# speedinghzl/DSRG

Measured on AMD Instinct MI355X. Metric: images/sec DSRG train step (VGG16 321x321, 21-class), higher is better.
Workload: dtype bf16 backbone (fp32 master weights) + f32/f64 supervision path

## Files before the change

dsrg_amd/_lib.py:

```python
import ctypes
import os

import torch

_HERE = os.path.dirname(os.path.abspath(__file__))
LIB_PATH = os.path.join(_HERE, os.environ.get("DSRG_LIB") or "libdsrg_hip.so")

OK, ERR_INVALID, ERR_HIP, ERR_UNSUPPORTED, ERR_NOMEM = 0, -1, -2, -3, -4


class DsrgError(RuntimeError):
    def __init__(self, code, msg):
        RuntimeError.__init__(self, "libdsrg_hip error %d: %s" % (code, msg))
        self.code = code


class CrfParams(ctypes.Structure):
    _fields_ = [("w_bilateral", ctypes.c_float), ("theta_alpha_x", ctypes.c_float),
                ("theta_alpha_y", ctypes.c_float), ("theta_beta_r", ctypes.c_float),
                ("theta_beta_g", ctypes.c_float), ("theta_beta_b", ctypes.c_float),
                ("w_gaussian", ctypes.c_float), ("theta_gamma_x", ctypes.c_float),
                ("theta_gamma_y", ctypes.c_float), ("n_iters", ctypes.c_int32)]

    @classmethod
# ... 60 lines not shown
    "dsrg_flush_reductions": (_i, [_vp]),
    "dsrg_conv_igemm_residual_bf16": (_i, [_vp] * 6 + [_i] * 8 + [_vp]),
    "dsrg_conv_igemm_split_f32": (_i, [_vp, _vp, _vp, _vp] + [_i] * 8 + [_vp]),
    "dsrg_add_relu_bf16": (_i, [_vp, _vp, _vp, _sz, _vp]),
    "dsrg_relu_mask_bf16": (_i, [_vp, _vp, _vp, _vp, _sz, _vp]),
    "dsrg_bias_grad_bf16": (_i, [_vp, _vp, _vp, _i, ctypes.c_long, _i, _vp]),
    "dsrg_heads_forward_bf16": (_i, [_vp, _i, _vp, _vp, _vp, _i, _i, _i, _i, _vp]),
    "dsrg_conv3x3_direct_bf16": (_i, [_vp, _vp, _vp, _vp, _i, _i, _i, _i, _i, _i, _vp]),
    "dsrg_conv3x3_direct_dgrad_workspace": (_sz, [_i]),
    "dsrg_conv3x3_direct_dgrad_bf16": (_i, [_vp] * 6 + [_sz] + [_i] * 5 + [_vp]),
    "dsrg_conv_igemm_supported": (_i, [_i, _i, _i]),
    "dsrg_conv_igemm_bf16": (_i, [_vp, _vp, _vp, _vp, _vp, _i, _i, _i, _i, _i, _i, _i, _i, ctypes.c_float, ctypes.c_ulonglong, _vp, _sz,
                                  _vp]),
    "dsrg_conv_igemm_workspace": (_sz, []),
    "dsrg_conv_igemm_dgrad_workspace": (_sz, [_i] * 5),
    "dsrg_conv_igemm_dgrad_bf16": (_i, [_vp] * 6 + [_i] * 7 + [_f, _vp, _sz, _vp]),
    "dsrg_conv_igemm_workspace_status": (_i, [_vp, _vp, _vp]),
    "dsrg_pack_conv_weight_f32": (_i, [_vp, _vp, _vp, _i, _i, _i, _vp]),
    "dsrg_sgd_pack_f32": (_i, [_i] + [_vp] * 9 + [_f, _vp]),
    "dsrg_conv_igemm_wgrad_workspace": (_sz, [_i, _i, _i, _i, _i, _i, _i]),
    "dsrg_conv_igemm_wgrad_bf16": (_i, [_vp, _vp, _vp, _vp, _i, _vp, _sz, _i, _i, _i, _i, _i, _i, _i, _vp]),
    "dsrg_conv_igemm_backward_bf16": (_i, [_vp, _vp, _vp, _vp, _vp, _vp, _i, _vp, _f, _vp, ctypes.c_size_t, _vp, ctypes.c_size_t, _i, _i, _i, _i, _i, _i, _vp]),
    "dsrg_conv3x3_wgrad_workspace": (_sz, [_i, _i, _i, _i, _i]),
    "dsrg_conv3x3_wgrad_bf16": (_i, [_vp, _vp, _vp, _vp, _sz, _i, _i, _i, _i, _i, _vp]),
    "dsrg_conv3x3_wgrad_f32": (_i, [_vp, _vp, _vp, _vp, _sz, _i, _i, _i, _i, _i, _vp]),
    "dsrg_pack_conv_weight_direct_f32": (_i, [_vp, _vp, _vp, _i, _i, _vp]),
    "dsrg_heads_backward_chunks": (_i, [_i]),
    "dsrg_heads_backward_bf16": (_i, [_vp, _i, _vp, _vp, _vp, _sz, _vp, _vp, _i, _i, _i, _i, _vp]),
    "dsrg_heads_backward_relu_workspace": (_sz, [_i] * 3),
    "dsrg_heads_backward_relu_bf16": (_i, [_vp, _i, _vp, _vp, _vp, _sz, _vp, _vp, _f, _vp, _vp, _sz] + [_i] * 4 + [_vp]),
    "dsrg_maxpool3x3_fwd_bf16": (_i, [_vp, _vp, _vp, _i, _i, _i, _i, _i, _i, _i, _vp]),
    "dsrg_maxpool3x3_relu_fwd_bf16": (_i, [_vp, _vp, _vp, _i, _i, _i, _i, _i, _i, _i, _vp]),
    "dsrg_maxpool3x3_bwd_bf16": (_i, [_vp, _vp, _vp, _i, _i, _i, _i, _i, _i, _i, _vp]),
    "dsrg_maxpool3x3_bwd_relu_bf16": (_i, [_vp, _vp, _vp, _vp, _vp, _vp, _i, _i, _i, _i, _i, _i, _i, _vp]),
    "dsrg_supervision_step": (_i, [_vp, _i, _vp, _vp, _i, _i, _vp, _vp, _d, _d, ctypes.POINTER(CrfParams),
                                   _vp, _vp, _vp, _vp, _vp, _vp]),
}

_LIB = None


def lib():
    global _LIB
    if _LIB is None:
        if not os.path.exists(LIB_PATH):
            raise ImportError(
                "%s is missing — build it with `make -C dsrg_amd/csrc` (hipcc --offload-arch=gfx950) or "
                "`python -c 'import __graft_entry__ as g; g.build()'`.  There is no CPU fallback." % LIB_PATH)
        L = ctypes.CDLL(LIB_PATH)
        for name, (res, args) in SIGNATURES.items():
            fn = getattr(L, name)
            fn.restype = res
            fn.argtypes = args
        _LIB = L
    return _LIB


def check(rc):
    if rc != OK:
        raise DsrgError(rc, lib().dsrg_last_error().decode("utf-8", "replace"))


def require_gpu():
    if lib().dsrg_device_count() < 1:
        raise DsrgError(ERR_HIP, "no HIP device visible — the DSRG supervision kernels need an MI355X "
                                 "(gfx950); there is no CPU fallback")
# ... 1 lines not shown
```

dsrg_amd/backbone.py:

```python
import torch
import torch.nn as nn
import torch.nn.functional as F


import os as _os
_WGRAD_MIN_COUT = int(_os.environ.get("DSRG_WGRAD_MIN_COUT", "512"))
_DIRECT_CONV = _os.environ.get("DSRG_DIRECT_CONV", "1")
_DIRECT_C3 = _os.environ.get("DSRG_DIRECT_C3", "1") == "1"
_DIRECT_FN = _os.environ.get("DSRG_DIRECT_FN", "1") == "1"
_FUSE_POOL = _os.environ.get("DSRG_FUSE_POOL", "1") == "1"
_GEMM_1X1_BWD = _os.environ.get("DSRG_GEMM_1X1_BWD", "1") == "1"
_DIRECT_WGRAD = _os.environ.get("DSRG_DIRECT_WGRAD", "1") == "1"
_GEMM_DGRAD_MAX_MAP = int(_os.environ.get("DSRG_GEMM_DGRAD_MAX_MAP", "2048"))
_WGRAD_T = _os.environ.get("DSRG_WGRAD_T", "1") == "1"
_IGEMM = _os.environ.get("DSRG_IGEMM", "1") == "1"
_FC7_IGEMM = _os.environ.get("DSRG_FC7_IGEMM", "1") == "1"


def _im2col_gemm(x, weight, bias, dilation, relu, want_cols=False):
    B, C, H, W = x.shape
    cout, k = weight.shape[0], weight.shape[2]
    xn = x.permute(0, 2, 3, 1)
    if not xn.is_contiguous():
        xn = xn.contiguous()
# ... 434 lines not shown

class FusedDropout(nn.Identity):
    """placeholder for the Dropout layer that runs inside the GemmConv2d two slots in front of it (`fuse_dropout`)"""


class _MaxPool3x3Fn(torch.autograd.Function):
    @staticmethod
    def forward(ctx, x, stride, ceil_mode):
        from .ops import maxpool3x3_fwd
        out, code = maxpool3x3_fwd(x, stride, ceil_mode)
        ctx.save_for_backward(code)
        ctx.in_shape, ctx.stride = x.shape, stride
        return out

    @staticmethod
    def backward(ctx, g):
        from .ops import maxpool3x3_bwd
        (code,) = ctx.saved_tensors
        return maxpool3x3_bwd(g, code, ctx.in_shape, ctx.stride), None, None


class _AvgPool3x3Fn(torch.autograd.Function):
    @staticmethod
    def forward(ctx, x):
        from .ops import avgpool3x3_s1
        return avgpool3x3_s1(x)

    @staticmethod
    def backward(ctx, g):
        from .ops import avgpool3x3_s1
        return avgpool3x3_s1(g)


class AvgPool3x3(nn.AvgPool2d):

    def __init__(self):
        super().__init__(3, 1, 1)

    def forward(self, x):
        if x.is_cuda and x.dtype == torch.bfloat16 and x.shape[1] % 8 == 0 and \
                x.is_contiguous(memory_format=torch.channels_last):
            return _AvgPool3x3Fn.apply(x)
        if x.is_cuda and x.dim() == 4 and not x.is_contiguous():
            x = x.contiguous()
        return super().forward(x)


class MaxPool3x3(nn.MaxPool2d):

    def __init__(self, stride, ceil_mode=False):
        super().__init__(3, stride, 1, ceil_mode=ceil_mode)

    def forward(self, x):
        if x.is_cuda and x.dtype == torch.bfloat16 and x.shape[1] % 8 == 0 and \
                x.is_contiguous(memory_format=torch.channels_last):
            return _MaxPool3x3Fn.apply(x, self.stride, self.ceil_mode)
        return super().forward(x)


def _pool3x3(x, stride, ceil_mode):
    if x.is_cuda and x.dtype == torch.bfloat16 and x.shape[1] % 8 == 0 and x.is_contiguous(memory_format=torch.channels_last):
        return _MaxPool3x3Fn.apply(x, stride, ceil_mode)
    return F.max_pool2d(x, 3, stride, 1, ceil_mode=ceil_mode)


def _conv_relu(cin, cout, dilation=1, gemm=False, pool=None, chain=False):
# ... 39 lines not shown
    @staticmethod
    def backward(ctx, g):
        return tuple(g[i].as_strided(shape, stride) if g[i].is_contiguous() else g[i].reshape(shape)
                     for i, (shape, stride) in enumerate(ctx.layouts))


class VGG16ASPP(nn.Module):

    def __init__(self, num_classes=21, dropout=0.5, gemm_convs=True):
        super().__init__()
        L = []
        p2 = (2, True)
        L += _conv_relu(3, 64) + _conv_relu(64, 64, pool=p2, chain=True)
        L += _conv_relu(64, 128, 1, gemm_convs) + _conv_relu(128, 128, 1, gemm_convs, pool=p2, chain=True)
        L += _conv_relu(128, 256, 1, gemm_convs) + _conv_relu(256, 256, 1, gemm_convs, chain=True) + \
            _conv_relu(256, 256, 1, gemm_convs, pool=p2, chain=True)
        g = gemm_convs
        L += _conv_relu(256, 512, 1, g) + _conv_relu(512, 512, 1, g, chain=True) + _conv_relu(512, 512, 1, g, chain=True) + [MaxPool3x3(1)]
        L += _conv_relu(512, 512, 2, g) + _conv_relu(512, 512, 2, g, chain=True) + _conv_relu(512, 512, 2, g, chain=True) + [MaxPool3x3(1)]
        L += [AvgPool3x3()]
        self.features = nn.Sequential(*L)
        self.branches = nn.ModuleList()
        for d in (6, 12, 18, 24):
            g = gemm_convs
            fc8 = GemmConv2d(1024, num_classes, 1, gemm=g)
            nn.init.normal_(fc8.weight, std=0.01)
            nn.init.zeros_(fc8.bias)
            self.branches.append(nn.Sequential(
                GemmConv2d(512, 1024, 3, padding=d, dilation=d, fuse_relu=True, gemm=g, fuse_dropout=dropout), FusedReLU(),
                FusedDropout(),
                GemmConv2d(1024, 1024, 1, fuse_relu=True, gemm=g, fuse_dropout=dropout), FusedReLU(), FusedDropout(), fc8))

    def forward(self, x):
        f = self.features(x)
        hs = []
        fc6 = [br[0] for br in self.branches]
        if len(fc6) <= 4 and all(_igemm_route(m, f, len(fc6)) and m.stride == (1, 1) and m.padding == m.dilation for m in fc6):
            p = fc6[0].fuse_dropout if self.training else 0.0
            n = len(fc6)
            links = [_GradLink() for _ in range(n)] if torch.is_grad_enabled() else None
            hs = list(_IgemmConvFn.apply(3, [m.dilation[0] for m in fc6], True, p, None, n, None, links, *([f] * n),
                                         *[m.weight for m in fc6], *[m.bias for m in fc6]))
            fc7 = [br[3] for br in self.branches]
            if all(isinstance(m, GemmConv2d) and m.kernel_size == (1, 1) and m.fuse_relu and m.bias is not None and m.gemm
                   and m.in_channels % 256 == 0 and m.out_channels % 256 == 0 for m in fc7):
                p7 = fc7[0].fuse_dropout if self.training else 0.0
                links7 = [_GradLink() for _ in range(n)] if torch.is_grad_enabled() else None
                hs = list(_IgemmConvFn.apply(1, [1] * n, True, p7, None, n, links, links7, *hs, *[m.weight for m in fc7],
                                             *[m.bias for m in fc7]))
                for h, lk in zip(hs, links7 or []):
                    h._dsrg_grad_link = lk
            else:
                for i, br in enumerate(self.branches):
                    for m in list(br)[1:-1]:
                        hs[i] = m(hs[i])
        else:
            for br in self.branches:
                h = f
                for m in list(br)[:-1]:
                    h = m(h)
                hs.append(h)
        heads = [br[-1] for br in self.branches]
        if hs[0].is_cuda and hs[0].dtype == torch.bfloat16 and len(hs) <= 4 and heads[0].out_channels <= 32 \
                and heads[0].in_channels % 256 == 0:
            w = _StackKernels.apply(*[m.weight for m in heads])
            b = torch.stack([m.bias for m in heads])
            links = [getattr(h, "_dsrg_grad_link", None) for h in hs]
# ... 57 lines not shown
```

dsrg_amd/csrc/api.hip:

```cpp
#include <math.h>
#include <stdarg.h>
#include <stdio.h>
#include <string.h>
#include <mutex>
#include <new>
#include "common.h"

namespace dsrg {

static thread_local char g_err[512] = "";
int set_error(int code, const char *fmt, ...) {
    va_list ap;
    va_start(ap, fmt);
    vsnprintf(g_err, sizeof(g_err), fmt, ap);
    va_end(ap);
    return code;
}

static inline size_t align256(size_t x) { return (x + 255) & ~(size_t)255; }

}

using namespace dsrg;

// ... 603 lines not shown
extern "C" int dsrg_heads_backward_chunks(int M) { return heads_bwd_chunks(M); }
extern "C" int dsrg_heads_backward_bf16(const void *const *x_dev, int n_branches, const float *w_dev, const float *g_dev,
                                        void *gx_dev, size_t gx_branch_stride_bytes, float *gw_dev, float *partial_dev, int B,
                                        int HW, int K, int O, void *stream) {
    if (!x_dev || !w_dev || !g_dev || (!gx_dev && !gw_dev) || (gw_dev && !partial_dev) || B < 1 || HW < 1)
        return set_error(DSRG_ERR_INVALID, "bad argument");
    for (int k = 0; k < n_branches && k < 4; k++)
        if (!x_dev[k]) return set_error(DSRG_ERR_INVALID, "NULL branch input");
    return launch_heads_bwd(x_dev, n_branches, w_dev, g_dev, gx_dev, gx_branch_stride_bytes, gw_dev, partial_dev, B, HW, K, O,
                            static_cast<hipStream_t>(stream));
}
extern "C" size_t dsrg_heads_backward_relu_workspace(int n_branches, int M, int K) { return heads_bwd_relu_workspace(n_branches, M, K); }
extern "C" int dsrg_heads_backward_relu_bf16(const void *const *x_dev, int n_branches, const float *w_dev, const float *g_dev,
                                             void *gx_dev, size_t gx_branch_stride_bytes, float *gw_dev, float *partial_dev,
                                             float relu_scale, float *bias_grad_dev, void *workspace_dev, size_t workspace_bytes,
                                             int B, int HW, int K, int O, void *stream) {
    if (!x_dev || !w_dev || !g_dev || !gx_dev || (gw_dev && !partial_dev) || B < 1 || HW < 1 || !(relu_scale > 0.0f) || !bias_grad_dev)
        return set_error(DSRG_ERR_INVALID, "bad argument");
    for (int k = 0; k < n_branches && k < 4; k++)
        if (!x_dev[k]) return set_error(DSRG_ERR_INVALID, "NULL branch input");
    return launch_heads_bwd(x_dev, n_branches, w_dev, g_dev, gx_dev, gx_branch_stride_bytes, gw_dev, partial_dev, B, HW, K, O,
                            static_cast<hipStream_t>(stream), relu_scale, bias_grad_dev, workspace_dev, workspace_bytes);
}
extern "C" int dsrg_maxpool3x3_fwd_bf16(const void *in, void *out, void *code, int B, int H, int W, int OH, int OW, int C,
                                        int stride, void *stream) {
    if (!in || !out || !code) return set_error(DSRG_ERR_INVALID, "NULL argument");
    return launch_maxpool3x3_fwd(in, out, code, B, H, W, OH, OW, C, stride, static_cast<hipStream_t>(stream));
}
extern "C" int dsrg_maxpool3x3_relu_fwd_bf16(const void *in, void *out, void *code, int B, int H, int W, int OH, int OW, int C,
                                             int stride, void *stream) {
    if (!in || !out || !code) return set_error(DSRG_ERR_INVALID, "NULL argument");
    return launch_maxpool3x3_fwd(in, out, code, B, H, W, OH, OW, C, stride, static_cast<hipStream_t>(stream), true);
}
extern "C" int dsrg_maxpool3x3_bwd_bf16(const void *gout, const void *code, void *gin, int B, int H, int W, int OH, int OW,
                                        int C, int stride, void *stream) {
    if (!gout || !code || !gin) return set_error(DSRG_ERR_INVALID, "NULL argument");
    return launch_maxpool3x3_bwd(gout, code, gin, B, H, W, OH, OW, C, stride, static_cast<hipStream_t>(stream));
}

extern "C" int dsrg_maxpool3x3_bwd_relu_bf16(const void *gout, const void *code, const void *relu_out, void *gin, float *bias_grad,
                                             float *partials, int partial_blocks, int B, int H, int W, int OH, int OW, int C,
                                             void *stream) {
    if (!gout || !code || !gin || !bias_grad || !partials) return set_error(DSRG_ERR_INVALID, "NULL argument");
    return launch_maxpool3x3_bwd_relu(gout, code, relu_out, gin, bias_grad, partials, partial_blocks, B, H, W, OH, OW, C,
                                      static_cast<hipStream_t>(stream));
}

extern "C" int dsrg_supervision_step(dsrg_ctx_t c, int B, const float *logits, const float *images, int img_h,
                                     int img_w, const float *labels, const float *cues, double th1, double th2,
                                     const dsrg_crf_params *prm, float *losses, float *grad_logits,
                                     float *probs_out, float *seeds_out, float *logq_out, void *stream) {
    if (!c || !logits || !labels || !cues || !losses || !grad_logits)
        return set_error(DSRG_ERR_INVALID, "NULL argument");
    if (B < 1 || B > c->maxB) return set_error(DSRG_ERR_INVALID, "batch %d outside 1..%d", B, c->maxB);
    const bool prepared = images == nullptr;
    {
        int prc = check_params(prm);
        if (prc) return prc;
    }
    if (!prepared && (img_h < 1 || img_w < 1)) return set_error(DSRG_ERR_INVALID, "bad image size");
    if (prepared) {
        if (c->prepared_B != B || memcmp(&c->prepared_prm, prm, offsetof(dsrg_crf_params, n_iters)) != 0)
            return set_error(DSRG_ERR_INVALID, "images_dev is NULL but dsrg_crf_prepare_batch was not called "
                                               "for this batch size / these kernel parameters");
    }
    hipStream_t s = static_cast<hipStream_t>(stream);
// ... 228 lines not shown
```

dsrg_amd/csrc/backbone_ops.hip:

```cpp
#include "common.h"
#include <algorithm>
#ifndef DSRG_EXP
#define DSRG_EXP 0
#endif
#include <cstdlib>
#include <cstring>

namespace dsrg {

__device__ __forceinline__ float bf16_lo(uint32_t w) { return __uint_as_float(w << 16); }
__device__ __forceinline__ float bf16_hi(uint32_t w) { return __uint_as_float(w & 0xffff0000u); }
__device__ __forceinline__ uint32_t f32_to_bf16_rne(float f) {
    uint32_t u = __float_as_uint(f);
    if ((u & 0x7fffffffu) > 0x7f800000u) return (u >> 16) | 0x40u;
    return (u + 0x7fffu + ((u >> 16) & 1u)) >> 16;
}
__device__ __forceinline__ uint32_t pack_bf16(float lo, float hi) { return f32_to_bf16_rne(lo) | (f32_to_bf16_rne(hi) << 16); }

constexpr int kRbThreads = 256;

__global__ __launch_bounds__(kRbThreads) void relu_bwd_bias_kernel(const uint4 *__restrict__ g, const uint4 *__restrict__ y,
                                                                    uint4 *__restrict__ gm, float *__restrict__ part,
                                                                    int rows, int C8, int rows_per_block, float scale) {
    __shared__ float red[kRbThreads][9];
// ... 320 lines not shown
    size_t r = idx / C8;
    const int x = (int)(r % W);
    r /= W;
    const int y = (int)(r % H);
    const int b = (int)(r / H);
    float acc[8] = {0.f, 0.f, 0.f, 0.f, 0.f, 0.f, 0.f, 0.f};
#pragma unroll
    for (int dy = -1; dy <= 1; ++dy) {
        const int yy = y + dy;
        if (yy < 0 || yy >= H) continue;
#pragma unroll
        for (int dx = -1; dx <= 1; ++dx) {
            const int xx = x + dx;
            if (xx < 0 || xx >= W) continue;
            const uint4 v = in[(((size_t)b * H + yy) * W + xx) * C8 + c];
            const uint32_t w[4] = {v.x, v.y, v.z, v.w};
#pragma unroll
            for (int k = 0; k < 4; ++k) { acc[2 * k] += bf16_lo(w[k]); acc[2 * k + 1] += bf16_hi(w[k]); }
        }
    }
#pragma unroll
    for (int k = 0; k < 8; ++k) acc[k] = acc[k] / 9.0f;
    out[idx] = make_uint4(pack_bf16(acc[0], acc[1]), pack_bf16(acc[2], acc[3]), pack_bf16(acc[4], acc[5]), pack_bf16(acc[6], acc[7]));
}
int launch_avgpool3x3_s1(const void *in, void *out, int B, int H, int W, int C, hipStream_t stream) {
    if (C % 8 != 0) return set_error(DSRG_ERR_UNSUPPORTED, "avgpool3x3: channels must be a multiple of 8");
    if (B <= 0 || H <= 0 || W <= 0) return set_error(DSRG_ERR_INVALID, "avgpool3x3: bad shape");
    const size_t total = (size_t)B * H * W * (C / 8);
    hipLaunchKernelGGL(avgpool3x3_s1_kernel, dim3((unsigned)((total + 255) / 256)), dim3(256), 0, stream, (const uint4 *)in,
                       (uint4 *)out, B, H, W, C / 8);
    DSRG_LAUNCH_CHECK();
    return DSRG_OK;
}

__global__ __launch_bounds__(256) void add_relu_kernel(const uint4 *__restrict__ a, const uint4 *__restrict__ b, uint4 *__restrict__ y, size_t n8) {
    const size_t i = (size_t)blockIdx.x * 256 + threadIdx.x;
    if (i >= n8) return;
    const uint4 va = a[i], vb = b[i];
    const uint32_t wa[4] = {va.x, va.y, va.z, va.w}, wb[4] = {vb.x, vb.y, vb.z, vb.w};
    uint32_t o[4];
#pragma unroll
    for (int k = 0; k < 4; k++)
        o[k] = pack_bf16(fmaxf(bf16_lo(wa[k]) + bf16_lo(wb[k]), 0.0f), fmaxf(bf16_hi(wa[k]) + bf16_hi(wb[k]), 0.0f));
    y[i] = make_uint4(o[0], o[1], o[2], o[3]);
}
__global__ __launch_bounds__(256) void relu_mask_kernel(const uint4 *__restrict__ g, const uint4 *__restrict__ g2, const uint4 *__restrict__ y,
                                                        uint4 *__restrict__ gm, size_t n8) {
    const size_t i = (size_t)blockIdx.x * 256 + threadIdx.x;
    if (i >= n8) return;
    const uint4 vg = g[i], vy = y[i];
    uint32_t wg[4] = {vg.x, vg.y, vg.z, vg.w};
    const uint32_t wy[4] = {vy.x, vy.y, vy.z, vy.w};
    if (g2) {
        const uint4 v2 = g2[i];
        const uint32_t w2[4] = {v2.x, v2.y, v2.z, v2.w};
#pragma unroll
        for (int k = 0; k < 4; k++) wg[k] = pack_bf16(bf16_lo(wg[k]) + bf16_lo(w2[k]), bf16_hi(wg[k]) + bf16_hi(w2[k]));
    }
#pragma unroll
    for (int k = 0; k < 4; k++)
        wg[k] &= ((int16_t)(wy[k] & 0xffffu) > 0 ? 0x0000ffffu : 0u) | ((int32_t)wy[k] >= 0x10000 ? 0xffff0000u : 0u);
    gm[i] = make_uint4(wg[0], wg[1], wg[2], wg[3]);
}
int launch_add_relu(const void *a, const void *b, void *y, size_t n, hipStream_t stream) {
    if (n == 0 || n % 8) return set_error(DSRG_ERR_INVALID, "add_relu: element count must be a positive multiple of 8");
    hipLaunchKernelGGL(add_relu_kernel, dim3((unsigned)((n / 8 + 255) / 256)), dim3(256), 0, stream, (const uint4 *)a, (const uint4 *)b,
// ... 787 lines not shown
```

dsrg_amd/csrc/common.h:

```cpp
#pragma once
#include <hip/hip_runtime.h>
#include <stdint.h>
#include <stddef.h>
#include <atomic>
#include "../../include/dsrg_hip.h"

namespace dsrg {

int set_error(int code, const char *fmt, ...);
#define DSRG_HIP_CHECK(expr)                                                              \
    do {                                                                                  \
        hipError_t _e = (expr);                                                           \
        if (_e != hipSuccess)                                                             \
            return ::dsrg::set_error(DSRG_ERR_HIP, "%s failed: %s (%s:%d)", #expr,        \
                                     hipGetErrorString(_e), __FILE__, __LINE__);          \
    } while (0)
#define DSRG_LAUNCH_CHECK() DSRG_HIP_CHECK(hipGetLastError())

__device__ __forceinline__ void colsum_block(const float *__restrict__ p, float *__restrict__ out, int rows, int cout, int bx, float (*red)[64]) {
    const int cl = threadIdx.x & 63, c = bx * 64 + cl, q = threadIdx.x >> 6;
    float s0 = 0.0f, s1 = 0.0f;
    int r = q;
    for (; r + 16 < rows; r += 32) {
        s0 += p[(size_t)r * cout + c];
// ... 175 lines not shown
                            int relu, hipStream_t stream);
int launch_conv_igemm(const void *const *x, const void *const *w, const float *const *bias, void *const *y, const int *dil,
                      int ngroups, int B, int H, int W, int cin, int cout, int k, int relu, float drop_p, unsigned long long seed,
                      void *workspace, size_t workspace_bytes, hipStream_t stream, const void *const *mask = nullptr,
                      float out_scale = 1.0f, float *const *colsum = nullptr, void *colsum_ws = nullptr, size_t colsum_ws_bytes = 0);
size_t conv_igemm_colsum_workspace(int ngroups, int B, int H, int W, int cout);
size_t conv_igemm_workspace();
int conv_igemm_workspace_status(const void *workspace, hipStream_t stream, int *status);
size_t conv_igemm_wgrad_workspace(int ngroups, int B, int H, int W, int cin, int cout, int k);
int launch_conv_igemm_wgrad(const void *const *x, const void *const *g, void *const *gw, const int *dil, int ngroups, void *workspace,
                            size_t workspace_bytes, int B, int H, int W, int cin, int cout, int k, int out_bf16, hipStream_t stream);
int launch_pack_conv_weight(const float *w, void *fwd, void *dgrad, int cout, int cin, int k, hipStream_t stream, int plain = 0,
                            const float *scale = nullptr);
int launch_conv_igemm_backward_residual(const void *g, const void *wd, const void *x, const void *mask, const void *res, void *gx, void *gw,
                                        const float *gw_scale, int dil, void *wgrad_ws, size_t wgrad_ws_bytes, int B, int H, int W, int cin,
                                        int cout, int k, hipStream_t stream);
int heads_bwd_chunks(int M);
int launch_heads_bwd(const void *const *x, int nbr, const float *w, const float *g, void *gx, size_t gx_branch_stride,
                     float *gw, float *partial, int B, int HW, int K, int O, hipStream_t stream, float relu_scale = 0.0f,
                     float *bias_grad = nullptr, void *colsum_ws = nullptr, size_t colsum_ws_bytes = 0);
size_t heads_bwd_relu_workspace(int nbr, int M, int K);
int launch_add_relu(const void *a, const void *b, void *y, size_t n, hipStream_t stream);
int launch_aspp_shift_sum(const void *yp, const float *bias, float *out, const int *offsets, int J, int O, int CT, int B, int H, int W,
                          hipStream_t stream);
int launch_aspp_shift_gather(const float *g, void *gp, const int *offsets, int J, int O, int CT, int B, int H, int W, hipStream_t stream);
int launch_relu_mask(const void *g, const void *g2, const void *y, void *gm, size_t n, hipStream_t stream);
int launch_igemm_colsum(const float *const *parts, float *const *outs, int ngroups, int rows, int cout, hipStream_t stream);
int launch_maxpool3x3_bwd_relu(const void *gout, const void *code, const void *y, void *gin, float *bias_grad, float *part,
                                int part_blocks, int B, int H, int W, int OH, int OW, int C, hipStream_t stream);
int launch_maxpool3x3_fwd(const void *in, void *out, void *code, int B, int H, int W, int OH, int OW, int C, int stride,
                          hipStream_t stream, bool relu_in = false);
int launch_maxpool3x3_bwd(const void *gout, const void *code, void *gin, int B, int H, int W, int OH, int OW, int C,
                          int stride, hipStream_t stream);

#ifdef __HIPCC__
__device__ __forceinline__ float exp_cr(float x) { return (float)exp((double)x); }

using rsrc_t = decltype(__builtin_amdgcn_make_buffer_rsrc((void *)nullptr, (short)0, 0, 0));
__device__ __forceinline__ rsrc_t make_rsrc(const void *p, size_t bytes) {
    const uint64_t a = reinterpret_cast<uint64_t>(p);
    const uint32_t lo = __builtin_amdgcn_readfirstlane((uint32_t)a);
    const uint32_t hi = __builtin_amdgcn_readfirstlane((uint32_t)(a >> 32));
    const uint32_t nb = __builtin_amdgcn_readfirstlane((uint32_t)bytes);
    void *q = reinterpret_cast<void *>(((uint64_t)hi << 32) | lo);
    return __builtin_amdgcn_make_buffer_rsrc(q, (short)0, (int)nb, 0x00020000);
}
__device__ __forceinline__ uint32_t ld_u32(rsrc_t r, uint32_t voff, uint32_t soff = 0) {
    return __builtin_amdgcn_raw_buffer_load_b32(r, voff, soff, 0);
}
__device__ __forceinline__ float ld_f32(rsrc_t r, uint32_t voff, uint32_t soff = 0) {
    return __uint_as_float(__builtin_amdgcn_raw_buffer_load_b32(r, voff, soff, 0));
}
__device__ __forceinline__ uint32_t ld_u16(rsrc_t r, uint32_t voff, uint32_t soff = 0) {
    return (uint32_t)__builtin_amdgcn_raw_buffer_load_b16(r, voff, soff, 0);
}
template <int U>
__device__ __forceinline__ void stage16_to_lds(unsigned char *dst, const void *src, uint32_t nbytes, int tid) {
    using v4 = decltype(__builtin_amdgcn_raw_buffer_load_b128(rsrc_t(), 0, 0, 0));
    const rsrc_t r = make_rsrc(src, nbytes);
    for (uint32_t base = 0; base < nbytes; base += 1024u * 16u * U) {
        v4 x[U];
#pragma unroll
        for (int u = 0; u < U; u++) x[u] = __builtin_amdgcn_raw_buffer_load_b128(r, (uint32_t)tid * 16u, base + (uint32_t)u * (1024u * 16u), 0);
#pragma unroll
        for (int u = 0; u < U; u++) {
            const uint32_t off = base + (uint32_t)u * (1024u * 16u) + (uint32_t)tid * 16u;
// ... 12 lines not shown
```

dsrg_amd/ops.py:

```python
import ctypes
import threading

import torch

from . import _lib
from ._lib import CrfParams, check


def _stream():
    return ctypes.c_void_p(torch.cuda.current_stream().cuda_stream)


def _ptr(t):
    return ctypes.c_void_p(t.data_ptr()) if t is not None else None


def _f32c(t, name):
    if not (t.is_cuda and t.dtype == torch.float32 and t.is_contiguous()):
        raise ValueError("%s must be a contiguous float32 CUDA tensor" % name)
    return t


_defer = [False]
_defer_keep = []


def _keep_until_flush(*tensors):
    if _defer[0]:
        _defer_keep.extend(t for t in tensors if t is not None)


@__import__("contextlib").contextmanager
def deferred_reductions(enabled=True):
# ... 955 lines not shown
    gw = torch.empty((n, O, K), dtype=torch.float32, device=g.device)
    part = torch.empty(L.dsrg_heads_backward_chunks(M) * n * O * K, dtype=torch.float32, device=g.device)
    ptrs = (ctypes.c_void_p * 4)(*([x.data_ptr() for x in xs] + [None] * (4 - n)))
    if relu_scale > 0.0 and need_gx:
        gb = torch.empty((n, K), dtype=torch.float32, device=g.device)
        ws = torch.empty(L.dsrg_heads_backward_relu_workspace(n, M, K), dtype=torch.uint8, device=g.device)
        _keep_until_flush(ws)
        check(L.dsrg_heads_backward_relu_bf16(ptrs, n, _ptr(weight), _ptr(g), _ptr(gx), M * K * 2, _ptr(gw), _ptr(part),
                                              float(relu_scale), _ptr(gb), _ptr(ws), ws.numel(), B, H * W, K, O, _stream()))
        return [gx[k].permute(0, 3, 1, 2) for k in range(n)], gw, gb
    check(L.dsrg_heads_backward_bf16(ptrs, n, _ptr(weight), _ptr(g), _ptr(gx), M * K * 2, _ptr(gw), _ptr(part), B, H * W, K, O,
                                     _stream()))
    return ([gx[k].permute(0, 3, 1, 2) for k in range(n)] if need_gx else None), gw


def maxpool3x3_out_size(n, stride, ceil_mode):
    num = n + 2 - 3
    o = (-(-num // stride) if ceil_mode else num // stride) + 1
    if (o - 1) * stride >= n + 1:
        o -= 1
    return o


def maxpool3x3_fwd(x, stride, ceil_mode, relu_input=False):
    B, C, H, W = x.shape
    OH, OW = maxpool3x3_out_size(H, stride, ceil_mode), maxpool3x3_out_size(W, stride, ceil_mode)
    out = torch.empty((B, C, OH, OW), dtype=x.dtype, device=x.device, memory_format=torch.channels_last)
    code = torch.empty((B, OH, OW, C), dtype=torch.uint8, device=x.device)
    fn = _lib.lib().dsrg_maxpool3x3_relu_fwd_bf16 if relu_input else _lib.lib().dsrg_maxpool3x3_fwd_bf16
    check(fn(_ptr(x), _ptr(out), _ptr(code), B, H, W, OH, OW, C, stride, _stream()))
    return out, code


def maxpool3x3_bwd(gout, code, in_shape, stride):
    B, C, H, W = in_shape
    OH, OW = gout.shape[2], gout.shape[3]
    gout = gout.contiguous(memory_format=torch.channels_last)
    gin = torch.empty((B, C, H, W), dtype=gout.dtype, device=gout.device, memory_format=torch.channels_last)
    check(_lib.lib().dsrg_maxpool3x3_bwd_bf16(_ptr(gout), _ptr(code), _ptr(gin), B, H, W, OH, OW, C, stride, _stream()))
    return gin


def maxpool3x3_bwd_relu(gout, code, relu_out, stride=2, gb_out=None):
    have_y = torch.is_tensor(relu_out)
    B, C, H, W = relu_out.shape if have_y else relu_out
    OH, OW = gout.shape[2], gout.shape[3]
    cl = torch.channels_last
    if stride != 2 or not (gout.is_cuda and gout.dtype == torch.bfloat16 and C % 8 == 0 and 256 % (C // 8) == 0) or (
            have_y and not (relu_out.is_cuda and relu_out.dtype == torch.bfloat16 and relu_out.is_contiguous(memory_format=cl))):
        raise ValueError("maxpool3x3_bwd_relu: stride 2, bf16 channels_last, channels / 8 a divisor of 256")
    gout = gout.contiguous(memory_format=cl)
    gin = torch.empty((B, C, H, W), dtype=torch.bfloat16, device=gout.device, memory_format=cl)
    gb = _dest(gb_out, (C,), torch.float32, gout.device)
    part = _partial_rows(gout.device, C)
    check(_lib.lib().dsrg_maxpool3x3_bwd_relu_bf16(_ptr(gout), _ptr(code), _ptr(relu_out) if have_y else None, _ptr(gin), _ptr(gb), _ptr(part),
                                                   _PARTIAL_BLOCKS, B, H, W, OH, OW, C, _stream()))
    return gin, gb


class DSRGSupervision(torch.autograd.Function):

    @staticmethod
    def forward(ctx, logits, images, labels, cues, th1, th2, scale_factor, maxiter, prepared=False):
        losses, grad, _ = supervision_step(logits.contiguous(), images, labels, cues, th1, th2, scale_factor, maxiter,
                                           prepared=prepared)
        ctx.save_for_backward(grad)
        ctx.mark_non_differentiable(losses)
        return losses.sum(), losses

    @staticmethod
    def backward(ctx, g_total, _g_losses):
        (grad,) = ctx.saved_tensors
# ... 7 lines not shown
```

include/dsrg_hip.h:

```cpp
#ifndef DSRG_HIP_H
#define DSRG_HIP_H

#include <stddef.h>
#include <stdint.h>

#ifdef __cplusplus
extern "C" {
#endif

#pragma GCC visibility push(default)

#define DSRG_OK 0
#define DSRG_ERR_INVALID (-1)
#define DSRG_ERR_HIP (-2)
#define DSRG_ERR_UNSUPPORTED (-3)
#define DSRG_ERR_NOMEM (-4)

const char *dsrg_last_error(void);
int dsrg_device_count(void);
int dsrg_host_register(void *host, size_t bytes);
int dsrg_host_unregister(void *host);

typedef struct dsrg_crf_s *dsrg_crf_t;

// ... 131 lines not shown
                                     int ksize, void *stream);
int dsrg_sgd_pack_f32(int n, float *const *param_dev, const float *const *grad_dev, float *const *momentum_dev, void *const *fwd_dev,
                      void *const *dgrad_dev, const int *shape, const long long *numel, const float *lr, const float *weight_decay,
                      float momentum, void *stream);
size_t dsrg_conv_igemm_wgrad_workspace(int ngroups, int B, int H, int W, int cin, int cout, int ksize);
int dsrg_conv_igemm_wgrad_bf16(const void *const *x_dev, const void *const *g_dev, void *const *gw_dev, const int *dilation,
                               int ngroups, void *workspace_dev, size_t workspace_bytes, int B, int H, int W, int cin, int cout,
                               int ksize, int out_bf16, void *stream);
int dsrg_conv_igemm_backward_bf16(const void *g_dev, const void *w_dgrad_dev, const void *x_dev, const void *mask_dev, void *gx_dev,
                                  float *gw_dev, int dilation, float *bias_grad_dev, float mask_scale, void *colsum_workspace_dev,
                                  size_t colsum_workspace_bytes, void *wgrad_workspace_dev, size_t wgrad_workspace_bytes, int B, int H,
                                  int W, int cin, int cout, int ksize, void *stream);
int dsrg_conv_igemm_backward_residual_bf16(const void *g_dev, const void *w_dgrad_dev, const void *x_dev, const void *mask_dev,
                                           const void *res_dev, void *gx_dev, float *gw_dev, const float *gw_scale_dev, int dilation,
                                           void *wgrad_workspace_dev, size_t wgrad_workspace_bytes, int B, int H, int W, int cin, int cout,
                                           int ksize, void *stream);
int dsrg_heads_forward_bf16(const void *const *x_dev, int n_branches, const float *w_dev, const float *bias_dev,
                            float *out_dev, int B, int HW, int K, int O, void *stream);
int dsrg_heads_backward_chunks(int M);
int dsrg_heads_backward_bf16(const void *const *x_dev, int n_branches, const float *w_dev, const float *g_dev,
                             void *gx_dev, size_t gx_branch_stride_bytes, float *gw_dev, float *partial_dev, int B,
                             int HW, int K, int O, void *stream);
size_t dsrg_heads_backward_relu_workspace(int n_branches, int M, int K);
int dsrg_heads_backward_relu_bf16(const void *const *x_dev, int n_branches, const float *w_dev, const float *g_dev,
                                  void *gx_dev, size_t gx_branch_stride_bytes, float *gw_dev, float *partial_dev,
                                  float relu_scale, float *bias_grad_dev, void *workspace_dev, size_t workspace_bytes, int B,
                                  int HW, int K, int O, void *stream);
int dsrg_maxpool3x3_fwd_bf16(const void *in_dev, void *out_dev, void *code_dev, int B, int H, int W, int OH, int OW, int C,
                             int stride, void *stream);
int dsrg_maxpool3x3_relu_fwd_bf16(const void *in_dev, void *out_dev, void *code_dev, int B, int H, int W, int OH, int OW, int C,
                                  int stride, void *stream);
int dsrg_maxpool3x3_bwd_bf16(const void *gout_dev, const void *code_dev, void *gin_dev, int B, int H, int W, int OH, int OW,
                             int C, int stride, void *stream);
int dsrg_maxpool3x3_bwd_relu_bf16(const void *gout_dev, const void *code_dev, const void *relu_out_dev, void *gin_dev,
                                  float *bias_grad_dev, float *partials_dev, int partial_blocks, int B, int H, int W, int OH,
                                  int OW, int C, void *stream);

int dsrg_supervision_step(dsrg_ctx_t ctx, int B, const float *logits_dev, const float *images_dev,
                          int img_h, int img_w, const float *labels_dev, const float *cues_dev,
                          double th1, double th2, const dsrg_crf_params *params,
                          float *losses_dev, float *grad_logits_dev,
                          float *probs_dev, float *seeds_dev, float *logq_dev, void *stream);

#pragma GCC visibility pop

#ifdef __cplusplus
}
#endif
#endif
```

Baseline: 1969.

## Fuse stride-1 maxpool and avgpool backward into one LDS-tiled kernel

Adds an LDS-tiled backward kernel for the stride-1 3x3 maxpool. It can also fold in the preceding avgpool3x3 backward, so the avgpool gradient is computed in shared memory and never written to global memory. The forward pass detects MaxPool(s1)+AvgPool pairs in the VGG feature stack and routes them through a fused autograd function, and plain stride-1 maxpool backward also switches to the tiled kernel. This removes one full-resolution gradient round-trip and one launch, at the cost of halo recomputation and LDS-limited occupancy with the default 7x7 tiles.

```diff
diff --git a/dsrg_amd/_lib.py b/dsrg_amd/_lib.py
--- a/dsrg_amd/_lib.py
+++ b/dsrg_amd/_lib.py
@@ -116,6 +116,7 @@
     "dsrg_maxpool3x3_fwd_bf16": (_i, [_vp, _vp, _vp, _i, _i, _i, _i, _i, _i, _i, _vp]),
     "dsrg_maxpool3x3_relu_fwd_bf16": (_i, [_vp, _vp, _vp, _i, _i, _i, _i, _i, _i, _i, _vp]),
     "dsrg_maxpool3x3_bwd_bf16": (_i, [_vp, _vp, _vp, _i, _i, _i, _i, _i, _i, _i, _vp]),
+    "dsrg_maxpool3x3_s1_tiled_bwd_bf16": (_i, [_vp, _vp, _vp] + [_i] * 7 + [_vp]),
     "dsrg_maxpool3x3_bwd_relu_bf16": (_i, [_vp, _vp, _vp, _vp, _vp, _vp, _i, _i, _i, _i, _i, _i, _i, _vp]),
     "dsrg_supervision_step": (_i, [_vp, _i, _vp, _vp, _i, _i, _vp, _vp, _d, _d, ctypes.POINTER(CrfParams),
                                    _vp, _vp, _vp, _vp, _vp, _vp]),
diff --git a/dsrg_amd/backbone.py b/dsrg_amd/backbone.py
--- a/dsrg_amd/backbone.py
+++ b/dsrg_amd/backbone.py
@@ -490,6 +490,46 @@
         return avgpool3x3_s1(g)
 
 
+class _MaxAvgPool3x3Fn(torch.autograd.Function):
+
+    @staticmethod
+    def forward(ctx, x):
+        from .ops import maxpool3x3_fwd, avgpool3x3_s1
+        pooled, code = maxpool3x3_fwd(x, 1, False)
+        out = avgpool3x3_s1(pooled)
+        ctx.save_for_backward(code)
+        ctx.in_shape = x.shape
+        return out
+
+    @staticmethod
+    def backward(ctx, g):
+        from .ops import maxavgpool3x3_s1_bwd
+        (code,) = ctx.saved_tensors
+        return maxavgpool3x3_s1_bwd(g, code)
+
+
+def _no_hooks(*mods):
+    return not any(m._forward_hooks or m._forward_pre_hooks or m._backward_hooks for m in mods)
+
+
+def _run_features(features, x):
+    from . import ops
+    if not _no_hooks(features):
+        return features(x)
+    mods = list(features)
+    i = 0
+    while i < len(mods):
+        m = mods[i]
+        if isinstance(m, MaxPool3x3) and m.stride == 1 and not m.ceil_mode and i + 1 < len(mods) and \
+                type(mods[i + 1]) is AvgPool3x3 and ops._FUSED_POOLS and ops.pool_tiled_ok(x) and _no_hooks(m, mods[i + 1]):
+            x = _MaxAvgPool3x3Fn.apply(x)
+            i += 2
+            continue
+        x = m(x)
+        i += 1
+    return x
+
+
 class AvgPool3x3(nn.AvgPool2d):
 
     def __init__(self):
@@ -595,7 +635,7 @@
                 GemmConv2d(1024, 1024, 1, fuse_relu=True, gemm=g, fuse_dropout=dropout), FusedReLU(), FusedDropout(), fc8))
 
     def forward(self, x):
-        f = self.features(x)
+        f = _run_features(self.features, x)
         hs = []
         fc6 = [br[0] for br in self.branches]
         if len(fc6) <= 4 and all(_igemm_route(m, f, len(fc6)) and m.stride == (1, 1) and m.padding == m.dilation for m in fc6):
diff --git a/dsrg_amd/csrc/api.hip b/dsrg_amd/csrc/api.hip
--- a/dsrg_amd/csrc/api.hip
+++ b/dsrg_amd/csrc/api.hip
@@ -659,6 +659,11 @@
     if (!in || !out || !code) return set_error(DSRG_ERR_INVALID, "NULL argument");
     return launch_maxpool3x3_fwd(in, out, code, B, H, W, OH, OW, C, stride, static_cast<hipStream_t>(stream), true);
 }
+extern "C" int dsrg_maxpool3x3_s1_tiled_bwd_bf16(const void *gout, const void *code, void *gin, int B, int H, int W, int C, int avg,
+                                                 int tile_h, int tile_w, void *stream) {
+    if (!gout || !code || !gin) return set_error(DSRG_ERR_INVALID, "NULL argument");
+    return launch_maxpool3x3_s1_tiled_bwd(gout, code, gin, B, H, W, C, avg != 0, tile_h, tile_w, static_cast<hipStream_t>(stream));
+}
 extern "C" int dsrg_maxpool3x3_bwd_bf16(const void *gout, const void *code, void *gin, int B, int H, int W, int OH, int OW,
                                         int C, int stride, void *stream) {
     if (!gout || !code || !gin) return set_error(DSRG_ERR_INVALID, "NULL argument");
diff --git a/dsrg_amd/csrc/backbone_ops.hip b/dsrg_amd/csrc/backbone_ops.hip
--- a/dsrg_amd/csrc/backbone_ops.hip
+++ b/dsrg_amd/csrc/backbone_ops.hip
@@ -376,6 +376,149 @@
     DSRG_LAUNCH_CHECK();
     return DSRG_OK;
 }
+
+static int pool_check(int B, int H, int W, int OH, int OW, int C, int stride);
+constexpr int kPoolCG = 8;
+template <bool AVG>
+__global__ __launch_bounds__(256) void maxpool3x3_s1_tiled_bwd_kernel(const uint4 *__restrict__ gout, const uint2 *__restrict__ code,
+                                                                    uint4 *__restrict__ gin, int H, int W, int C8, int TH,
+                                                                    int TW, int tiles_x, int tiles_y) {
+    extern __shared__ uint4 pool_lds[];
+    int bid = blockIdx.x;
+    const int nch = C8 / kPoolCG;
+    const int cbase = (bid % nch) * kPoolCG;
+    bid /= nch;
+    const int tx = bid % tiles_x;
+    bid /= tiles_x;
+    const int ty = bid % tiles_y;
+    const int b = bid / tiles_y;
+    const int MH = TH + 2, MW = TW + 2;
+    const int y0 = ty * TH, x0 = tx * TW;
+    const int my0 = y0 - 1, mx0 = x0 - 1;
+    const int nm = MH * MW * kPoolCG;
+    uint4 *const gt = pool_lds;
+    uint2 *const ct = reinterpret_cast<uint2 *>(pool_lds + nm);
+    uint4 *const at = pool_lds + nm + (nm + 1) / 2;
+    if (AVG) {
+        const int AW = MW + 2, na = (MH + 2) * AW * kPoolCG;
+        for (int i0 = threadIdx.x; i0 < na; i0 += 4 * 256) {
+            uint4 v[4];
+#pragma unroll
+            for (int u = 0; u < 4; ++u) {
+                const int i = i0 + u * 256;
+                const int c = i % kPoolCG, p = i / kPoolCG;
+                const int yy = my0 - 1 + p / AW, xx = mx0 - 1 + p % AW;
+                v[u] = make_uint4(0u, 0u, 0u, 0u);
+                if (i < na && yy >= 0 && yy < H && xx >= 0 && xx < W) v[u] = gout[(((size_t)b * H + yy) * W + xx) * C8 + cbase + c];
+            }
+#pragma unroll
+            for (int u = 0; u < 4; ++u)
+                if (i0 + u * 256 < na) at[i0 + u * 256] = v[u];
+        }
+    }
+    for (int i0 = threadIdx.x; i0 < nm; i0 += 4 * 256) {
+        uint4 v[4];
+        uint2 cd[4];
+#pragma unroll
+        for (int u = 0; u < 4; ++u) {
+            const int i = i0 + u * 256;
+            const int c = i % kPoolCG, p = i / kPoolCG;
+            const int yy = my0 + p / MW, xx = mx0 + p % MW;
+            v[u] = make_uint4(0u, 0u, 0u, 0u);
+            cd[u] = make_uint2(0xffffffffu, 0xffffffffu);
+            if (i < nm && yy >= 0 && yy < H && xx >= 0 && xx < W) {
+                const size_t o = (((size_t)b * H + yy) * W + xx) * C8 + cbase + c;
+                cd[u] = code[o];
+                if (!AVG) v[u] = gout[o];
+            }
+        }
+#pragma unroll
+        for (int u = 0; u < 4; ++u)
+            if (i0 + u * 256 < nm) { ct[i0 + u * 256] = cd[u]; if (!AVG) gt[i0 + u * 256] = v[u]; }
+    }
+    __syncthreads();
+    if (AVG) {
+        const int AW = MW + 2;
+        for (int i = threadIdx.x; i < nm; i += 256) {
+            const int c = i % kPoolCG, p = i / kPoolCG;
+            const int my = p / MW, mx = p % MW;
+            const int y = my0 + my, x = mx0 + mx;
+            if (y < 0 || y >= H || x < 0 || x >= W) continue;
+            float acc[8] = {0.f, 0.f, 0.f, 0.f, 0.f, 0.f, 0.f, 0.f};
+#pragma unroll
+            for (int dy = -1; dy <= 1; ++dy) {
+                if (y + dy < 0 || y + dy >= H) continue;
+#pragma unroll
+                for (int dx = -1; dx <= 1; ++dx) {
+                    if (x + dx < 0 || x + dx >= W) continue;
+                    const uint4 v = at[((my + 1 + dy) * AW + mx + 1 + dx) * kPoolCG + c];
+                    const uint32_t w[4] = {v.x, v.y, v.z, v.w};
+#pragma unroll
+                    for (int k = 0; k < 4; ++k) { acc[2 * k] += bf16_lo(w[k]); acc[2 * k + 1] += bf16_hi(w[k]); }
+                }
+            }
+#pragma unroll
+            for (int k = 0; k < 8; ++k) acc[k] = acc[k] / 9.0f;
+            gt[i] = make_uint4(pack_bf16(acc[0], acc[1]), pack_bf16(acc[2], acc[3]), pack_bf16(acc[4], acc[5]), pack_bf16(acc[6], acc[7]));
+        }
+        __syncthreads();
+    }
+    for (int i = threadIdx.x; i < TH * TW * kPoolCG; i += 256) {
+        const int c = i % kPoolCG, p = i / kPoolCG;
+        const int ly = p / TW, lx = p % TW;
+        const int y = y0 + ly, x = x0 + lx;
+        if (y >= H || x >= W) continue;
+        float acc[8] = {0.f, 0.f, 0.f, 0.f, 0.f, 0.f, 0.f, 0.f};
+#pragma unroll
+        for (int dy = 0; dy < 3; ++dy) {
+            const int oy = y + 1 - dy;
+            if (oy < 0 || oy >= H) continue;
+#pragma unroll
+            for (int dx = 0; dx < 3; ++dx) {
+                const int ox = x + 1 - dx;
+                if (ox < 0 || ox >= W) continue;
+                const int m = ((ly + 2 - dy) * MW + lx + 2 - dx) * kPoolCG + c;
+                const uint2 cd = ct[m];
+                const uint4 gv = gt[m];
+                const uint32_t want = 3 * dy + dx;
+                const uint32_t gw[4] = {gv.x, gv.y, gv.z, gv.w};
+#pragma unroll
+                for (int k = 0; k < 4; ++k) {
+                    const uint32_t cw = k < 2 ? cd.x : cd.y;
+                    const uint32_t c0 = (cw >> (16 * (k & 1))) & 0xffu, c1 = (cw >> (16 * (k & 1) + 8)) & 0xffu;
+                    if (c0 == want) acc[2 * k] += bf16_lo(gw[k]);
+                    if (c1 == want) acc[2 * k + 1] += bf16_hi(gw[k]);
+                }
+            }
+        }
+        gin[(((size_t)b * H + y) * W + x) * C8 + cbase + c] =
+            make_uint4(pack_bf16(acc[0], acc[1]), pack_bf16(acc[2], acc[3]), pack_bf16(acc[4], acc[5]), pack_bf16(acc[6], acc[7]));
+    }
+}
+
+int launch_maxpool3x3_s1_tiled_bwd(const void *gout, const void *code, void *gin, int B, int H, int W, int C, bool avg, int TH,
+                                   int TW, hipStream_t stream) {
+    int rc = pool_check(B, H, W, H, W, C, 1);
+    if (rc) return rc;
+    if (C % (8 * kPoolCG) != 0) return set_error(DSRG_ERR_UNSUPPORTED, "pool3x3_tiled: channels must be a multiple of %d", 8 * kPoolCG);
+    if (TH <= 0 || TW <= 0) { TH = 7; TW = 7; }
+    if (TH > 64 || TW > 64) return set_error(DSRG_ERR_INVALID, "pool3x3_tiled: bad tile %d x %d", TH, TW);
+    const size_t nm = (size_t)(TH + 2) * (TW + 2) * kPoolCG;
+    const size_t lds = (nm + (nm + 1) / 2 + (avg ? (size_t)(TH + 4) * (TW + 4) * kPoolCG : 0)) * sizeof(uint4);
+    if (lds > 64 * 1024) return set_error(DSRG_ERR_INVALID, "pool3x3_tiled: tile %d x %d needs %zu bytes of LDS", TH, TW, lds);
+    const int tiles_x = (W + TW - 1) / TW, tiles_y = (H + TH - 1) / TH;
+    const long nblk = (long)B * tiles_y * tiles_x * (C / 8 / kPoolCG);
+    if (nblk > 0x7fffffffL) return set_error(DSRG_ERR_INVALID, "pool3x3_tiled: too many blocks");
+    if (avg)
+        hipLaunchKernelGGL(maxpool3x3_s1_tiled_bwd_kernel<true>, dim3((unsigned)nblk), dim3(256), lds, stream, (const uint4 *)gout,
+                           (const uint2 *)code, (uint4 *)gin, H, W, C / 8, TH, TW, tiles_x, tiles_y);
+    else
+        hipLaunchKernelGGL(maxpool3x3_s1_tiled_bwd_kernel<false>, dim3((unsigned)nblk), dim3(256), lds, stream, (const uint4 *)gout,
+                           (const uint2 *)code, (uint4 *)gin, H, W, C / 8, TH, TW, tiles_x, tiles_y);
+    DSRG_LAUNCH_CHECK();
+    return DSRG_OK;
+}
+
 
 __global__ __launch_bounds__(256) void add_relu_kernel(const uint4 *__restrict__ a, const uint4 *__restrict__ b, uint4 *__restrict__ y, size_t n8) {
     const size_t i = (size_t)blockIdx.x * 256 + threadIdx.x;
diff --git a/dsrg_amd/csrc/common.h b/dsrg_amd/csrc/common.h
--- a/dsrg_amd/csrc/common.h
+++ b/dsrg_amd/csrc/common.h
@@ -231,6 +231,8 @@
                           hipStream_t stream, bool relu_in = false);
 int launch_maxpool3x3_bwd(const void *gout, const void *code, void *gin, int B, int H, int W, int OH, int OW, int C,
                           int stride, hipStream_t stream);
+int launch_maxpool3x3_s1_tiled_bwd(const void *gout, const void *code, void *gin, int B, int H, int W, int C, bool avg, int TH,
+                                   int TW, hipStream_t stream);
 
 #ifdef __HIPCC__
 __device__ __forceinline__ float exp_cr(float x) { return (float)exp((double)x); }
diff --git a/dsrg_amd/ops.py b/dsrg_amd/ops.py
--- a/dsrg_amd/ops.py
+++ b/dsrg_amd/ops.py
@@ -1,4 +1,5 @@
 import ctypes
+import os
 import threading
 
 import torch
@@ -1020,12 +1021,36 @@
     return out, code
 
 
-def maxpool3x3_bwd(gout, code, in_shape, stride):
+_FUSED_POOLS = os.environ.get("DSRG_FUSED_POOLS", "1") != "0"
+
+
+def pool_tiled_ok(x):
+    return x.is_cuda and x.dtype == torch.bfloat16 and x.shape[1] % 64 == 0 and x.is_contiguous(memory_format=torch.channels_last)
+
+
+def maxpool3x3_bwd(gout, code, in_shape, stride, tiled=None, tile=(0, 0)):
     B, C, H, W = in_shape
     OH, OW = gout.shape[2], gout.shape[3]
     gout = gout.contiguous(memory_format=torch.channels_last)
     gin = torch.empty((B, C, H, W), dtype=gout.dtype, device=gout.device, memory_format=torch.channels_last)
+    if tiled is None:
+        tiled = _FUSED_POOLS and stride == 1 and pool_tiled_ok(gout)
+    if tiled:
+        check(_lib.lib().dsrg_maxpool3x3_s1_tiled_bwd_bf16(_ptr(gout), _ptr(code), _ptr(gin), B, H, W, C, 0, int(tile[0]),
+                                                           int(tile[1]), _stream()))
+        return gin
     check(_lib.lib().dsrg_maxpool3x3_bwd_bf16(_ptr(gout), _ptr(code), _ptr(gin), B, H, W, OH, OW, C, stride, _stream()))
+    return gin
+
+
+def maxavgpool3x3_s1_bwd(gout, code, tile=(0, 0)):
+    gout = gout.contiguous(memory_format=torch.channels_last)
+    if not pool_tiled_ok(gout):
+        raise ValueError("maxavgpool3x3_s1_bwd needs a bf16 CUDA tensor with 64 | channels")
+    B, C, H, W = gout.shape
+    gin = torch.empty_like(gout, memory_format=torch.channels_last)
+    check(_lib.lib().dsrg_maxpool3x3_s1_tiled_bwd_bf16(_ptr(gout), _ptr(code), _ptr(gin), B, H, W, C, 1, int(tile[0]), int(tile[1]),
+                                                       _stream()))
     return gin
 
 
diff --git a/include/dsrg_hip.h b/include/dsrg_hip.h
--- a/include/dsrg_hip.h
+++ b/include/dsrg_hip.h
@@ -187,6 +187,8 @@
                                   int stride, void *stream);
 int dsrg_maxpool3x3_bwd_bf16(const void *gout_dev, const void *code_dev, void *gin_dev, int B, int H, int W, int OH, int OW,
                              int C, int stride, void *stream);
+int dsrg_maxpool3x3_s1_tiled_bwd_bf16(const void *gout_dev, const void *code_dev, void *gin_dev, int B, int H, int W, int C,
+                                      int avg, int tile_h, int tile_w, void *stream);
 int dsrg_maxpool3x3_bwd_relu_bf16(const void *gout_dev, const void *code_dev, const void *relu_out_dev, void *gin_dev,
                                   float *bias_grad_dev, float *partials_dev, int partial_blocks, int B, int H, int W, int OH,
                                   int OW, int C, void *stream);
```

Result: no change. 1973, median of 6 (+0.2%).
